# rgovindjee/mpconstellation

Measured on AMD Instinct MI355X. Metric: satellite-MPC-steps/sec (whole constellation; 1 step = discretize + constraint terms + solve per SCP iteration; inputs and results resident in HBM -- value_pcie is the same step with H2D of the inputs and D2H of the results inside), higher is better.
Workload: dtype f64

## Files before the change

### mpconstellation_amd/csrc/solve_phases.hpp

```cpp
#pragma once

namespace MPCX_NS {
#ifdef MPCX_TWO_WAVE
using namespace mpcx;
#endif

struct ResAcc {
    double dual_max, prim_max, sq, zsum, lsum, prod_min, prod_max, prod_sum;
    double g_tf;
};

struct SatData {
    double aT[8][7], bT[8];
    int nT, linvt;
    int fixed_tf;
    int shared;
    double tS, rS;
    double w_vt, gh_vt, zeta_vt;
    double b_u, b_rmax, b_rmin, b_rfmax, b_tf[2], vt_des, w_tr, w_nu, tfbar;
    double WxK[49];
    double WxKsoft[49], gxKsoft[7];
    double ta[NTERM][7], tw[NTERM], tgh[NTERM], twin[NTERM];
    double avt[7], Hv[36], cv, gam, Wtf, gtf, sigmax;
    double Mb[NBD][NBD];
    double Sb[NBD][NBD];
    double siglam[NCH], xK[NCH][7];
    double sol[NBD];
    double zeta[NTERM];
    double red[8];
    double gl[3][GL_N];
    ResAcc racc[2];
    double rs_gtf, rs_rvt, rs_gex[NTERM];
    int dir_finite;
    struct Drv {
        double mu, dw_last, E0, delta_w, alpha, tau, mu_cur, rn0, mu_clip;
        double nz, nzl;
        int n_acc, status, it_count, n_reg, first_reg, mono, refined_prev, n_small, iter, have_dir, have_trial, clean, ls;
        double tol, acc_tol;
        int acc_iter, max_iter, n_refine;
    } dv;
    static constexpr int DRV_D0 = 3, DRV_I0 = 8;
    double infeas;
    double eps_r;
    int flag;
#ifdef MPCX_PHASE_TIMING
    unsigned long long fpt[16];
#endif
};

static_assert(offsetof(SatData::Drv, mu) == 0 && offsetof(SatData::Drv, E0) == (SatData::DRV_D0 - 1) * sizeof(double) &&
              offsetof(SatData::Drv, n_small) - offsetof(SatData::Drv, n_acc) == (SatData::DRV_I0 - 1) * sizeof(int) &&
              offsetof(SatData::Drv, status) - offsetof(SatData::Drv, n_acc) == sizeof(int) &&
              offsetof(SatData::Drv, first_reg) - offsetof(SatData::Drv, n_acc) == 4 * sizeof(int), "field order of the loop state's start values");

__device__ __forceinline__ double relax(double b) { return b + kBoundRelax * fmax(1.0, fabs(b)); }

__device__ __forceinline__ double wave_max(double v)
{
#pragma unroll
    for (int o = 32; o > 0; o >>= 1) v = fmax(v, __shfl_xor(v, o, 64));
    return v;
}
__device__ __forceinline__ double wave_min(double v)
{
#pragma unroll
    for (int o = 32; o > 0; o >>= 1) v = fmin(v, __shfl_xor(v, o, 64));
    return v;
}
__device__ __forceinline__ double wave_sum(double v)
{
#pragma unroll
    for (int o = 32; o > 0; o >>= 1) v += __shfl_xor(v, o, 64);
    return v;
}

__device__ __forceinline__ double gshfl8(double v, int q)
{
    switch (q) {
    case 0: return bcast8<0>(v);
    case 1: return bcast8<1>(v);
    case 2: return bcast8<2>(v);
    case 3: return bcast8<3>(v);
    case 4: return bcast8<4>(v);
    case 5: return bcast8<5>(v);
    case 6: return bcast8<6>(v);
    default: return bcast8<7>(v);
    }
}

__device__ __forceinline__ void wsync()
{
    __builtin_amdgcn_fence(__ATOMIC_ACQ_REL, "wavefront");
    __builtin_amdgcn_wave_barrier();
}

__device__ __forceinline__ int uni(int v) { return __builtin_amdgcn_readfirstlane(v); }
__device__ __forceinline__ double uni(double v)
{
    const unsigned long long u = (unsigned long long)__double_as_longlong(v);
    const unsigned lo = __builtin_amdgcn_readfirstlane((unsigned)u), hi = __builtin_amdgcn_readfirstlane((unsigned)(u >> 32));
    return __longlong_as_double((long long)(((unsigned long long)hi << 32) | lo));
}

__device__ void vt_reduced(const double *x, double vt_des, double &c, double *g6, double *H36)
{
    const double *r = x, *v = x + 3;
    const double q = r[0] * r[0] + r[1] * r[1] + r[2] * r[2];
    const double rv = r[0] * v[0] + r[1] * v[1] + r[2] * v[2];
    const double iq = 1.0 / q, iq2 = iq * iq, iq3 = iq2 * iq;
    c = v[0] * v[0] + v[1] * v[1] + v[2] * v[2] - rv * rv * iq - vt_des * vt_des;
    if (!g6) return;
    for (int i = 0; i < 3; ++i) {
        g6[i] = -2.0 * rv * v[i] * iq + 2.0 * rv * rv * r[i] * iq2;
        g6[3 + i] = 2.0 * v[i] - 2.0 * rv * r[i] * iq;
    }
    if (!H36) return;
    for (int i = 0; i < 3; ++i)
        for (int j = 0; j < 3; ++j) {
            const double I = (i == j) ? 1.0 : 0.0;
            const double Hvv = 2.0 * I - 2.0 * r[i] * r[j] * iq;
            const double Hrr = -2.0 * v[i] * v[j] * iq + 4.0 * rv * (v[i] * r[j] + r[i] * v[j]) * iq2 +
                               2.0 * rv * rv * I * iq2 - 8.0 * rv * rv * r[i] * r[j] * iq3;
            const double Hrv = -2.0 * v[i] * r[j] * iq - 2.0 * rv * I * iq + 4.0 * rv * r[i] * r[j] * iq2;
            H36[i * 6 + j] = Hrr;
            H36[(3 + i) * 6 + 3 + j] = Hvv;
            H36[i * 6 + 3 + j] = Hrv;
            H36[(3 + j) * 6 + i] = Hrv;
        }
}

__device__ __noinline__ void build_terminal(const double *xK, double mu_grav, double r_des, const SolveOpts &o, SatData &sd)
{
    double r[3] = {xK[0], xK[1], xK[2]}, v[3] = {xK[3], xK[4], xK[5]}, h[3], rh[3], hh[3];
    const double rn = sqrt(r[0] * r[0] + r[1] * r[1] + r[2] * r[2]);
    h[0] = r[1] * v[2] - r[2] * v[1]; h[1] = r[2] * v[0] - r[0] * v[2]; h[2] = r[0] * v[1] - r[1] * v[0];
    const double hn = sqrt(h[0] * h[0] + h[1] * h[1] + h[2] * h[2]);
    for (int i = 0; i < 3; ++i) { rh[i] = r[i] / rn; hh[i] = h[i] / hn; }
    const double ihn = 1.0 / hn, ihn3 = 1.0 / (hn * hn * hn), irn = 1.0 / rn, irn3 = 1.0 / (rn * rn * rn);
    double Ph[9], hh3[9], nSv[9], Sr[9], Dr_h[9], Dv_h[9], Dr_r[9];
    for (int i = 0; i < 3; ++i)
        for (int j = 0; j < 3; ++j) {
            hh3[i * 3 + j] = ihn3 * (h[i] * h[j]);
            Ph[i * 3 + j] = (i == j ? ihn : 0.0) - hh3[i * 3 + j];
            Dr_r[i * 3 + j] = (i == j ? irn : 0.0) - irn3 * (r[i] * r[j]);
        }
    nSv[0] = 0; nSv[1] = v[2]; nSv[2] = -v[1]; nSv[3] = -v[2]; nSv[4] = 0; nSv[5] = v[0]; nSv[6] = v[1]; nSv[7] = -v[0]; nSv[8] = 0;
    Sr[0] = 0; Sr[1] = -r[2]; Sr[2] = r[1]; Sr[3] = r[2]; Sr[4] = 0; Sr[5] = -r[0]; Sr[6] = -r[1]; Sr[7] = r[0]; Sr[8] = 0;
    for (int i = 0; i < 3; ++i)
        for (int j = 0; j < 3; ++j) {
            double a = 0.0, b = 0.0;
            for (int l = 0; l < 3; ++l) { a += Ph[i * 3 + l] * nSv[l * 3 + j]; b += hh3[i * 3 + l] * Sr[l * 3 + j]; }
            Dr_h[i * 3 + j] = a;
            Dv_h[i * 3 + j] = (i == j ? ihn : 0.0) - b;
        }
    double DrVr[3], DrVn[3], DvVn[3];
    for (int j = 0; j < 3; ++j) {
        DrVr[j] = v[0] * Dr_r[j] + v[1] * Dr_r[3 + j] + v[2] * Dr_r[6 + j];
        DrVn[j] = v[0] * Dr_h[j] + v[1] * Dr_h[3 + j] + v[2] * Dr_h[6 + j];
        DvVn[j] = hh[j] + (v[0] * Dv_h[j] + v[1] * Dv_h[3 + j] + v[2] * Dv_h[6 + j]);
    }
    const double Vr = v[0] * rh[0] + v[1] * rh[1] + v[2] * rh[2];
    const double Vn = v[0] * hh[0] + v[1] * hh[1] + v[2] * hh[2];
    double gR[6] = {DrVr[0], DrVr[1], DrVr[2], rh[0], rh[1], rh[2]};
    double gN[6] = {DrVn[0], DrVn[1], DrVn[2], DvVn[0], DvVn[1], DvVn[2]};
    double gRbar = 0.0, gNbar = 0.0;
    for (int i = 0; i < 6; ++i) { gRbar += gR[i] * xK[i]; gNbar += gN[i] * xK[i]; }
    for (int i = 0; i < 8; ++i) { sd.bT[i] = 0.0; for (int j = 0; j < 7; ++j) sd.aT[i][j] = 0.0; }
    sd.linvt = o.linvt; sd.nT = o.linvt ? 8 : 6; sd.fixed_tf = o.fixed_tf | o.shared_tf; sd.shared = o.shared_tf;
    sd.w_vt = 0.0; sd.gh_vt = 0.0; sd.zeta_vt = 0.0;
    for (int j = 0; j < 3; ++j) sd.aT[0][j] = -rh[j];
    sd.bT[0] = relax(-(r_des - o.eps_r));
    for (int j = 0; j < 6; ++j) { sd.aT[1][j] = gR[j]; sd.aT[2][j] = -gR[j]; sd.aT[3][j] = gN[j]; sd.aT[4][j] = -gN[j]; }
    const double c0r = Vr - gRbar, c0n = Vn - gNbar;
    sd.bT[1] = relax(o.eps_vr - c0r); sd.bT[2] = relax(o.eps_vr + c0r);
    sd.bT[3] = relax(o.eps_vn - c0n); sd.bT[4] = relax(o.eps_vn + c0n);
    sd.aT[5][6] = -1.0; sd.bT[5] = relax(-o.min_mass);
    if (o.linvt) {
        double th[3] = {hh[1] * rh[2] - hh[2] * rh[1], hh[2] * rh[0] - hh[0] * rh[2], hh[0] * rh[1] - hh[1] * rh[0]};
        double nSrh[9] = {0, rh[2], -rh[1], -rh[2], 0, rh[0], rh[1], -rh[0], 0};
        double Shh[9] = {0, -hh[2], hh[1], hh[2], 0, -hh[0], -hh[1], hh[0], 0};
        double Dr_t[9], Dv_t[9];
        for (int i = 0; i < 3; ++i)
            for (int j = 0; j < 3; ++j) {
                double a = 0.0, b = 0.0, c = 0.0;
                for (int l = 0; l < 3; ++l) { a += nSrh[i * 3 + l] * Dr_h[l * 3 + j]; b += Shh[i * 3 + l] * Dr_r[l * 3 + j]; c += nSrh[i * 3 + l] * Dv_h[l * 3 + j]; }
                Dr_t[i * 3 + j] = a + b; Dv_t[i * 3 + j] = c;
            }
        const double Vt = v[0] * th[0] + v[1] * th[1] + v[2] * th[2];
        const double Vc = sqrt(mu_grav / rn);
        const double kc = -0.5 * sqrt(mu_grav) * pow(rn, -2.5);
        double gT[6], gbar = 0.0, DrVc_r = 0.0;
        for (int j = 0; j < 3; ++j) {
            gT[j] = v[0] * Dr_t[j] + v[1] * Dr_t[3 + j] + v[2] * Dr_t[6 + j];
            gT[3 + j] = th[j] + (v[0] * Dv_t[j] + v[1] * Dv_t[3 + j] + v[2] * Dv_t[6 + j]);
        }
        for (int i = 0; i < 6; ++i) gbar += gT[i] * xK[i];
        for (int j = 0; j < 3; ++j) { DrVc_r += kc * r[j] * r[j]; gT[j] -= kc * r[j]; }
        const double c0t = Vt - gbar - Vc + DrVc_r;
        for (int j = 0; j < 6; ++j) { sd.aT[6][j] = gT[j]; sd.aT[7][j] = -gT[j]; }
        sd.bT[6] = relax(o.eps_vt - c0t); sd.bT[7] = relax(o.eps_vt + c0t);
    }
    sd.b_u = relax(o.u_max * o.u_max);
    sd.b_rmax = relax(o.r_max * o.r_max);
    sd.b_rmin = relax(-o.r_min);
    sd.b_rfmax = relax((r_des + o.eps_r) * (r_des + o.eps_r));
    sd.b_tf[0] = relax(0.0); sd.b_tf[1] = relax(o.tf_max);
    sd.vt_des = sqrt(mu_grav / r_des);
    sd.w_tr = o.w_tr; sd.w_nu = o.w_nu;
}

__device__ __noinline__ void build_terminal_sat(const double *xK, double mu_grav, double r_des, const SolveOpts &o, const double *popts, int sat, SatData &sd)
{
    SolveOpts os = o;
    if (popts) {
// ... 658 lines not shown
            sigmax = fmax(sigmax, sig);
        }
        sd.Wtf = W; sd.gtf = g; sd.sigmax = sigmax;
    }
    WG_SYNC();
}

__device__ __noinline__ void combine_channels(const Sat &s_in, SatData &sd, int lane, bool first)
{
    double *const stg = stage_area();
    const Sat s = uniform_view(s_in);
    const int K = s.K, KP = s.KP;
    double sol[NBD];
#pragma unroll
    for (int j = 0; j < NBD; ++j) sol[j] = sd.sol[j];
    wf64 *dr = wave_uniform(s.dr);
    cwf64 *it = wave_uniform((cwf64 *)s.it);
    cgf64 *traj = wave_uniform((cgf64 *)s.traj);
    for (int k0 = 0; k0 < K; k0 += 32) {
        const int nk = (K - k0 < 32) ? K - k0 : 32;
        const int n = nk * TR_N;
        constexpr int CQ = 8;
        for (int e0 = 0; e0 < n; e0 += 64 * CQ) {
            double v[CQ];
            int slot[CQ];
#pragma unroll
            for (int q = 0; q < CQ; ++q) {
                const int e = e0 + 64 * q + lane;
                const int ec = (e < n) ? e : 0;
                const int kl = ec / TR_N, i = ec - kl * TR_N;
                cgf64 *tr = traj + (size_t)(k0 + kl) * NCH * TR_N + i;
                double acc = tr[0];
#pragma unroll
                for (int j = 0; j < NBD; ++j)
                    acc += sol[j] * tr[(1 + j) * TR_N];
                v[q] = acc; slot[q] = (e < n) ? i * CMB_LD + kl : -1;
            }
#pragma unroll
            for (int q = 0; q < CQ; ++q) if (slot[q] >= 0) stg[slot[q]] = v[q];
        }
        WG_SYNC();
        constexpr int NQ = DIR_N * 32 / 64;
        double curv[NQ], Dv[NQ], rv[NQ];
#pragma unroll
        for (int q = 0; q < NQ; ++q) {
            const int e = lane + 64 * q;
            const int i = e >> 5, kl = e & 31, k = k0 + kl;
            const int off = (i < T_U) ? I_X + i : (i < T_NU ? I_U + (i - T_U) : (i < T_LAM ? I_NU + (i - T_NU) : I_LAM + (i - T_LAM)));
            const int dst = off * KP + (kl < nk ? k : k0);
            const int kc = (kl < nk) ? k : k0, j = (i >= T_LAM) ? i - T_LAM : 0;
            curv[q] = first ? it[dst] : dr[dst];
            Dv[q] = s.nb[(size_t)kc * NB_N + N_D + j]; rv[q] = s.ch[(size_t)kc * CH_N + C_RHS + R_RHO + j];
        }
        CHUNK_END
#pragma unroll
        for (int q = 0; q < NQ; ++q) {
            const int e = lane + 64 * q;
            const int i = e >> 5, kl = e & 31, k = k0 + kl;
            const bool act = kl < nk && !(k == K - 1 && i >= T_NU);
            const int off = (i < T_U) ? I_X + i : (i < T_NU ? I_U + (i - T_U) : (i < T_LAM ? I_NU + (i - T_NU) : I_LAM + (i - T_LAM)));
            const int dst = off * KP + (kl < nk ? k : k0);
            const double cur = curv[q];
            const double base = first ? ((i >= T_LAM) ? -cur : 0.0) : cur;
            const int j = (i >= T_LAM) ? i - T_LAM : 0;
            const double val = (i >= T_LAM) ? fma(Dv[q], stg[(T_NU + j) * CMB_LD + kl], rv[q]) : stg[(i < T_LAM ? i : 0) * CMB_LD + kl];
            if (act) dr[dst] = base + val;
        }
        WG_SYNC();
    }
    if (lane == 0) {
        if (first) { s.drg[G_TF] = sd.sol[0]; s.drg[G_LVT] = sd.linvt ? 0.0 : -s.itg[G_LVT] + sd.sol[1]; }
        else { s.drg[G_TF] += sd.sol[0]; if (!sd.linvt) s.drg[G_LVT] += sd.sol[1]; }
        if (sd.linvt) sd.zeta_vt = (first ? 0.0 : sd.zeta_vt) + sd.sol[1];
        for (int t = 0; t < NTERM; ++t) sd.zeta[t] = (first ? 0.0 : sd.zeta[t]) + sd.sol[2 + t];
    }
    WG_SYNC();
}

__device__ __noinline__ void reduced_residual(const Sat &s, SatData &sd, int lane)
{
    double *const stg = stage_area();
    double rvt_rhs, gex[NTERM];
    const int K = s.K;
    double gtf_part = 0.0;
    const double dtf = s.drg[G_TF];
    double gin[NTERM], rvt_x;
    {
        const auto dKc = s.drn(K - 1);
        double dK[7];
#pragma unroll
        for (int i = 0; i < 7; ++i) dK[i] = dKc[I_X + i];
        double av = 0.0;
#pragma unroll
        for (int i = 0; i < 7; ++i) av += sd.avt[i] * dK[i];
        rvt_rhs = -sd.cv - av;
        rvt_x = rvt_rhs;
        if (sd.linvt) {
            const double wex = sd.w_vt - sd.gam;
            const bool on = wex > 0.0;
            rvt_x = -(sd.gh_vt * (sd.gam / sd.w_vt) + sd.gam * av + (on ? sd.zeta_vt : 0.0)) / sd.gam;
            rvt_rhs = on ? -(av - sd.zeta_vt / wex + sd.gh_vt / sd.w_vt) : 0.0;
        }
        for (int t = 0; t < NTERM; ++t) {
            double adx = 0.0;
#pragma unroll
            for (int i = 0; i < 7; ++i) adx += sd.ta[t][i] * dK[i];
            const double wex = sd.tw[t] - sd.twin[t];
            const double share = (sd.tw[t] > 0.0) ? sd.twin[t] / sd.tw[t] : 1.0;
            const bool on = wex > 0.0;
            gin[t] = sd.tgh[t] * share + sd.twin[t] * adx + (on ? sd.zeta[t] : 0.0);
            gex[t] = on ? (adx - sd.zeta[t] / wex + sd.tgh[t] / sd.tw[t]) * wex : 0.0;
        }
    }
    for (int k0 = 0; k0 < K; k0 += 64) {
      const int k = k0 + lane;
      double *rec = stg + lane * RHS_LD;
      if (k < K) {
        cwf64 *nb = s.nb + (size_t)k * NB_N;
        const auto ns = s.nsn(k);
        const auto p = s.itn(k), d = s.drn(k);
        const bool hp = (k >= 1), dyn = (k <= K - 2), term = (k == K - 1);
        const auto pm = p.node(hp ? -1 : 0), dm = d.node(hp ? -1 : 0), dn = d.node(dyn ? 1 : 0);
        double lt[7], ltm[7];
#pragma unroll
        for (int i = 0; i < 7; ++i) {
            const double a0 = p[I_LAM + i], a1 = d[I_LAM + i], b0 = pm[I_LAM + i], b1 = dm[I_LAM + i];
            lt[i] = dyn ? a0 + a1 : 0.0;
            ltm[i] = hp ? b0 + b1 : 0.0;
        }
        CHUNK_END
        double dx[7], du[3], dnu[7], nsgx[7], nsgu[3], w3[9], wu[9], sx[SX_N];
#pragma unroll
        for (int i = 0; i < 7; ++i) { dx[i] = d[I_X + i]; dnu[i] = d[I_NU + i]; nsgx[i] = ns[NS_GX + i]; }
#pragma unroll
        for (int i = 0; i < 3; ++i) { du[i] = d[I_U + i]; nsgu[i] = ns[NS_GU + i]; }
#pragma unroll
        for (int i = 0; i < 9; ++i) { w3[i] = nb[N_W3 + i]; wu[i] = nb[N_WU + i]; }
#pragma unroll
        for (int i = 0; i < SX_N; ++i) sx[i] = nb[N_SX + i];
        const double dg = nb[N_DIAG];
        CHUNK_END
        double gx[7], gu[3];
        if (hp) {
            if (term) {
#pragma unroll
                for (int i = 0; i < 7; ++i) {
                    double acc = sd.gxKsoft[i] + ltm[i];
#pragma unroll
                    for (int j = 0; j < 7; ++j) acc += sd.WxKsoft[i * 7 + j] * dx[j];
                    gx[i] = acc;
                }
            } else {
#pragma unroll
                for (int i = 0; i < 7; ++i) {
                    double acc = nsgx[i] + ltm[i];
                    if (i < 3) {
#pragma unroll
                        for (int j = 0; j < 3; ++j) acc += w3[i * 3 + j] * dx[j];
                    } else acc += dg * dx[i];
                    gx[i] = acc;
                }
            }
            if (term) {
                const double lvt = s.itg[G_LVT] + s.drg[G_LVT];
#pragma unroll
                for (int i = 0; i < 7; ++i) gx[i] += sd.avt[i] * lvt;
            }
        } else {
#pragma unroll
            for (int i = 0; i < 7; ++i) gx[i] = 0.0;
        }
#pragma unroll
        for (int i = 0; i < 3; ++i) {
            double acc = nsgu[i];
#pragma unroll
            for (int j = 0; j < 3; ++j) acc += wu[i * 3 + j] * du[j];
            gu[i] = acc;
        }
        {
            const double ex_x = sx[SX_EX], ex_u = sx[SX_EU];
            const double a0 = sx[SX_A], a1 = sx[SX_A + 1], a2 = sx[SX_A + 2];
            const double c0 = sx[SX_CU], c1 = sx[SX_CU + 1], c2 = sx[SX_CU + 2];
            const double px = ex_x * (a0 * dx[0] + a1 * dx[1] + a2 * dx[2]);
            const double pu = ex_u * (c0 * du[0] + c1 * du[1] + c2 * du[2]);
            if (hp && dyn) { gx[0] += px * a0; gx[1] += px * a1; gx[2] += px * a2; }
            gu[0] += pu * c0; gu[1] += pu * c1; gu[2] += pu * c2;
        }
        double sg[7], dnx[7], dnuu[3];
        {
            double bm[21];
            const auto Bm = s.Bpt(hp ? k - 1 : 0), Sg = s.Sigt(dyn ? k : 0);
#pragma unroll
            for (int e = 0; e < 21; ++e) bm[e] = Bm[e];
#pragma unroll
            for (int i = 0; i < 7; ++i) { sg[i] = Sg[i]; dnx[i] = dn[I_X + i]; }
#pragma unroll
            for (int i = 0; i < 3; ++i) dnuu[i] = dn[I_U + i];
            CHUNK_END
            if (hp) {
#pragma unroll
                for (int j = 0; j < 3; ++j) {
                    double acc = 0.0;
#pragma unroll
                    for (int i = 0; i < 7; ++i) acc += bm[i * 3 + j] * ltm[i];
                    gu[j] -= acc;
                }
            }
        }
        double aff[7], atl[7];
#pragma unroll
        for (int j = 0; j < 7; ++j) atl[j] = 0.0;
        {
            const auto A = s.At(dyn ? k : 0);
#pragma unroll
            for (int h = 0; h < 2; ++h) {
                const int r0 = h ? 4 : 0, r1 = h ? 7 : 4;
                double am[28];
#pragma unroll
                for (int i = r0; i < r1; ++i)
#pragma unroll
                    for (int j = 0; j < 7; ++j) am[(i - r0) * 7 + j] = A[i * 7 + j];
                CHUNK_END
#pragma unroll
                for (int i = r0; i < r1; ++i) {
#pragma unroll
                    for (int j = 0; j < 7; ++j) atl[j] += am[(i - r0) * 7 + j] * lt[i];
                    double acc = dnx[i] - sg[i] * dtf - dnu[i];
#pragma unroll
                    for (int j = 0; j < 7; ++j) acc -= am[(i - r0) * 7 + j] * dx[j];
                    aff[i] = acc;
                }
            }
        }
        if (dyn && hp) {
#pragma unroll
            for (int j = 0; j < 7; ++j) gx[j] -= atl[j];
        }
        {
            double bn[21], bp[21];
            const auto Bn = s.Bnt(dyn ? k : 0), Bp = s.Bpt(dyn ? k : 0);
#pragma unroll
            for (int e = 0; e < 21; ++e) { bn[e] = Bn[e]; bp[e] = Bp[e]; }
            CHUNK_END
#pragma unroll
            for (int j = 0; j < 3; ++j) {
                double acc = 0.0;
#pragma unroll
                for (int i = 0; i < 7; ++i) acc += bn[i * 3 + j] * lt[i];
                if (dyn) gu[j] -= acc;
            }
#pragma unroll
            for (int i = 0; i < 7; ++i) {
                double acc = aff[i];
#pragma unroll
                for (int j = 0; j < 3; ++j) acc -= bn[i * 3 + j] * du[j] + bp[i * 3 + j] * dnuu[j];
                aff[i] = acc;
            }
        }
        {
            double rho[7], dd[7], ee[7];
#pragma unroll
            for (int i = 0; i < 7; ++i) { rho[i] = ns[NS_RHO + i]; dd[i] = ns[NS_D + i]; ee[i] = ns[NS_E + i]; }
            CHUNK_END
            if (dyn) {
                double sl = 0.0;
#pragma unroll
                for (int i = 0; i < 7; ++i) {
                    rec[R_RHO + i] = rho[i] + dd[i] * dnu[i] - lt[i];
                    rec[R_AFF + i] = -ee[i] - aff[i];
                    sl += sg[i] * lt[i];
                }
                gtf_part -= sl;
            }
        }
        if (term) {
            for (int t = 0; t < NTERM; ++t) {
#pragma unroll
                for (int i = 0; i < 7; ++i) gx[i] += gin[t] * sd.ta[t][i];
            }
#pragma unroll
            for (int i = 0; i < 7; ++i) gx[i] -= sd.gam * rvt_x * sd.avt[i];
#pragma unroll
            for (int i = 0; i < 7; ++i) { rec[R_RHO + i] = 0.0; rec[R_AFF + i] = 0.0; }
        }
#pragma unroll
        for (int i = 0; i < 7; ++i) rec[R_GX + i] = gx[i];
#pragma unroll
        for (int i = 0; i < 3; ++i) rec[R_GU + i] = gu[i];
      }
      WG_SYNC();
      {
          const int nr = ((K - k0 < 64) ? K - k0 : 64) * RHS_N;
          wf64 *ch = s.ch + (size_t)k0 * CH_N + C_RHS;
          for (int e = lane; e < nr; e += 64) { const int kl = e / RHS_N, i = e - kl * RHS_N; ch[(size_t)kl * CH_N + i] = stg[kl * RHS_LD + i]; }
      }
      WG_SYNC();
    }
    sd.rs_gtf = sd.gtf + sd.Wtf * dtf + wave_sum(gtf_part);
    sd.rs_rvt = rvt_rhs;
#pragma unroll
    for (int t = 0; t < NTERM; ++t) sd.rs_gex[t] = gex[t];
    WG_SYNC();
}

__device__ __forceinline__ void first_rhs_scalars(SatData &sd)
{
    sd.rs_gtf = sd.gtf;
    sd.rs_rvt = sd.linvt ? -sd.gh_vt / sd.w_vt : -sd.cv;
    for (int t = 0; t < NTERM; ++t) {
        const double share = (sd.tw[t] > 0.0) ? sd.twin[t] / sd.tw[t] : 1.0;
        sd.rs_gex[t] = sd.tgh[t] * (1.0 - share);
    }
    wsync();
}

__device__ __noinline__ double finish_direction(const Sat &s, SatData &sd, double mu, double tau, int lane)
{
    const int K = s.K;
    double amax = 1.0, bad = 0.0;
#define CHK(v) { if (!(fabs(v) < 1e300)) bad = 1.0; }
    const double b_u = sd.b_u, b_rmax = sd.b_rmax, b_rmin = sd.b_rmin, w_nu = sd.w_nu;
#define LIM(v, dv) { const double v_ = (v), d_ = (dv); if (d_ < 0.0) amax = fmin(amax, -tau * v_ / d_); }
    const int half = HALF_OF(lane);
    const bool h0 = (half == 0);
    for (int k = NODE_OF(lane); k < K; k += 32) {
        const auto p = s.itn(k), d = s.drn(k);
        const auto rb = s.rbn(k);
        double x[7], dx[7], u[3], du[3], bs[6], rv[4][8];
#pragma unroll
        for (int i = 0; i < 7; ++i) { x[i] = p[I_X + i]; dx[i] = d[I_X + i]; }
#pragma unroll
        for (int i = 0; i < 3; ++i) { u[i] = p[I_U + i]; du[i] = d[I_U + i]; }
#pragma unroll
        for (int i = 0; i < 6; ++i) bs[i] = p[I_SU + i];
        const double rb0 = rb[0], rb1 = rb[1], rb2 = rb[2];
#pragma unroll
        for (int r = 0; r < 4; ++r) {
            const int iv = 4 * half + r;
            const int i = (iv < 7) ? iv : 6;
            rv[r][0] = p[I_NU + i]; rv[r][1] = p[I_T + i]; rv[r][2] = p[I_STP + i]; rv[r][3] = p[I_ZTP + i];
            rv[r][4] = p[I_STN + i]; rv[r][5] = p[I_ZTN + i]; rv[r][6] = d[I_NU + i]; rv[r][7] = d[I_LAM + i];
        }
        CHUNK_END
        {
#pragma unroll
            for (int i = 0; i < 7; ++i) CHK(dx[i]);
#pragma unroll
            for (int i = 0; i < 3; ++i) CHK(du[i]);
            {
                const PairDir q = pair_dir(bs[0], bs[1], u[0] * u[0] + u[1] * u[1] + u[2] * u[2] - b_u,
                                           2.0 * (u[0] * du[0] + u[1] * du[1] + u[2] * du[2]), mu);
                LIM(bs[0], q.ds); LIM(bs[1], q.dz);
            }
            if (k >= 1) {
                const PairDir q = pair_dir(bs[2], bs[3], x[0] * x[0] + x[1] * x[1] + x[2] * x[2] - b_rmax,
                                           2.0 * (x[0] * dx[0] + x[1] * dx[1] + x[2] * dx[2]), mu);
                LIM(bs[2], q.ds); LIM(bs[3], q.dz);
            }
            if (k >= 1 && k <= K - 2) {
                const PairDir q = pair_dir(bs[4], bs[5], -(rb0 * x[0] + rb1 * x[1] + rb2 * x[2]) - b_rmin,
                                           -(rb0 * dx[0] + rb1 * dx[1] + rb2 * dx[2]), mu);
                LIM(bs[4], q.ds); LIM(bs[5], q.dz);
            }
        }
        {
            const bool dyn = (k <= K - 2);
#pragma unroll
            for (int r = 0; r < 4; ++r) {
                const int iv = 4 * half + r;
                const bool valid = (iv < 7) && dyn;
                const double nu = rv[r][0], tt = rv[r][1], stp = rv[r][2], ztp = rv[r][3];
                const double stn = rv[r][4], ztn = rv[r][5], dnu = rv[r][6], dlam = rv[r][7];
                const L1Dir q = l1_dir(nu, tt, stp, ztp, stn, ztn, dnu, mu, w_nu);
                if (valid) {
                    CHK(dnu); CHK(dlam); CHK(q.dt);
                    LIM(stp, q.dstp); LIM(ztp, q.dztp);
                    LIM(stn, q.dstn); LIM(ztn, q.dztn);
                }
            }
        }
        if (h0 && k == K - 1) {
// ... 38 lines not shown
```

### mpconstellation_amd/csrc/solve_riccati.hpp

```cpp
#pragma once

namespace MPCX_NS {
__device__ __forceinline__ bool inv3_spd(const double *Q, double *Qi)
{
    const double a = Q[0], b = Q[1], c = Q[2], d = Q[4], e = Q[5], f = Q[8];
    const double d1 = a;
    const double r1 = rcp_pos(d1 > 0.0 ? d1 : 1.0);
    const double l21 = b * r1, l31 = c * r1;
    const double d2 = d - l21 * b;
    const double r2 = rcp_pos(d2 > 0.0 ? d2 : 1.0);
    const double t32 = e - l31 * b;
    const double l32 = t32 * r2;
    const double d3 = f - l31 * c - l32 * t32;
    const double r3 = rcp_pos(d3 > 0.0 ? d3 : 1.0);
    const bool ok = (d1 > 0.0) && (d2 > 0.0) && (d3 > 0.0);
    const double m31 = l21 * l32 - l31, m32 = -l32, m21 = -l21;
    Qi[0] = r1 + m21 * m21 * r2 + m31 * m31 * r3;
    Qi[1] = m21 * r2 + m31 * m32 * r3;
    Qi[2] = m31 * r3;
    Qi[4] = r2 + m32 * m32 * r3;
    Qi[5] = m32 * r3;
    Qi[8] = r3;
    Qi[3] = Qi[1]; Qi[6] = Qi[2]; Qi[7] = Qi[5];
    return ok;
// ... 948 lines not shown
        }
        wsync();
        FT_MARK(14)
    }
    siglam += __shfl_xor(siglam, 1, 8);
    siglam += __shfl_xor(siglam, 2, 8);
    siglam += __shfl_xor(siglam, 4, 8);
    if (act && r == 0) sd.siglam[c] = siglam;
    WG_SYNC();
}

__device__ __forceinline__ int border_channel(int q) { return q == NBD - 1 ? 1 : 2 + q; }
__device__ __forceinline__ double border_iw(const SatData &sd, int p, bool &eq)
{
    eq = (p == 0) && !sd.linvt;
    const double wex = (p == 0) ? (sd.linvt ? sd.w_vt - sd.gam : 0.0) : sd.tw[p - 1] - sd.twin[p - 1];
    return (!eq && wex > 0.0) ? 1.0 / wex : 0.0;
}

__device__ __noinline__ bool border_factor(SatData &sd, int lane)
{
    if (lane < NBD * NBD) {
        const int p = lane / NBD, q = lane - NBD * p;
        const int c = border_channel(q);
        double v;
        if (p < NBD - 1) {
            const double *a = (p == 0) ? sd.avt : sd.ta[p - 1];
            v = 0.0;
#pragma unroll
            for (int l = 0; l < 7; ++l) v += a[l] * sd.xK[c][l];
        } else v = (q == NBD - 1 ? sd.Wtf : 0.0) - sd.siglam[c];
        if (sd.fixed_tf && (p == NBD - 1 || q == NBD - 1)) v = (p == q) ? 1.0 : 0.0;
        sd.Mb[p][q] = v; sd.Sb[p][q] = v;
    }
    WG_SYNC();
    double S[NBD][NBD];
#pragma unroll
    for (int p = 0; p < NBD; ++p)
#pragma unroll
        for (int q = 0; q < NBD; ++q) S[p][q] = sd.Mb[p][q];
#pragma unroll
    for (int p = 0; p < NBD - 1; ++p) {
        bool eq;
        const double iw = border_iw(sd, p, eq);
        const bool on = iw > 0.0;
        if (eq) continue;
#pragma unroll
        for (int q = 0; q < NBD; ++q) if (!on && q != p) { S[p][q] = 0.0; S[q][p] = 0.0; }
        S[p][p] = on ? S[p][p] - iw : -1.0;
    }
    bool ok = true;
    double rd[NBD];
#pragma unroll
    for (int p = 0; p < NBD; ++p) {
        const double d = S[p][p];
        if (p == NBD - 1) { if (!(d > 0.0)) ok = false; } else if (!(d < 0.0)) ok = false;
        rd[p] = 1.0 / d;
#pragma unroll
        for (int i = p + 1; i < NBD; ++i) {
            const double m = S[i][p] * rd[p];
#pragma unroll
            for (int j = p + 1; j < NBD; ++j) S[i][j] -= m * S[p][j];
            S[i][p] = m;
        }
    }
    WG_SYNC();
    if (lane == 0) {
#pragma unroll
        for (int p = 0; p < NBD; ++p) {
            sd.Mb[p][p] = rd[p];
#pragma unroll
            for (int i = p + 1; i < NBD; ++i) sd.Mb[i][p] = S[i][p];
        }
    }
    WG_SYNC();
    return ok;
}

__device__ __noinline__ void border_solve(SatData &sd, int lane)
{
    const double gtf_rhs = sd.rs_gtf, rvt_rhs = sd.rs_rvt;
    const double *gex = sd.rs_gex;
    double rb[NBD], x[NBD], r[NBD];
#pragma unroll
    for (int p = 0; p < NBD - 1; ++p) {
        const double *a = (p == 0) ? sd.avt : sd.ta[p - 1];
        double acc = 0.0;
#pragma unroll
        for (int l = 0; l < 7; ++l) acc += a[l] * sd.xK[0][l];
        rb[p] = -acc;
    }
    rb[0] += rvt_rhs;
    double iw[NBD - 1];
    bool eqr[NBD - 1];
#pragma unroll
    for (int p = 0; p < NBD - 1; ++p) {
        iw[p] = border_iw(sd, p, eqr[p]);
        if (p >= 1) rb[p] = (iw[p] > 0.0) ? rb[p] - gex[p - 1] * iw[p] : 0.0;
        else if (!eqr[0] && !(iw[0] > 0.0)) rb[0] = 0.0;
    }
    rb[NBD - 1] = sd.fixed_tf ? 0.0 : -gtf_rhs + sd.siglam[0];
    auto ldl_solve = [&](double (&v)[NBD]) {
#pragma unroll
        for (int p = 0; p < NBD; ++p)
#pragma unroll
            for (int i = p + 1; i < NBD; ++i) v[i] -= sd.Mb[i][p] * v[p];
#pragma unroll
        for (int p = 0; p < NBD; ++p) v[p] *= sd.Mb[p][p];
#pragma unroll
        for (int p = NBD - 1; p >= 0; --p)
#pragma unroll
            for (int i = p + 1; i < NBD; ++i) v[p] -= sd.Mb[i][p] * v[i];
    };
#pragma unroll
    for (int p = 0; p < NBD; ++p) x[p] = rb[p];
    ldl_solve(x);
#pragma unroll
    for (int p = 0; p < NBD; ++p) {
        double acc = rb[p];
#pragma unroll
        for (int q = 0; q < NBD; ++q) {
            double s = sd.Sb[p][q];
            const int pc = p < NBD - 1 ? p : 0, qc = q < NBD - 1 ? q : 0;
            const bool zp = p < NBD - 1 && !eqr[pc], zq = q < NBD - 1 && !eqr[qc];
            const bool offp = zp && !(iw[pc] > 0.0), offq = zq && !(iw[qc] > 0.0);
            if (p == q && zp) s = offp ? -1.0 : s - iw[pc];
            else if (offp || offq) s = 0.0;
            acc -= s * x[q];
        }
        r[p] = acc;
    }
    ldl_solve(r);
#pragma unroll
    for (int p = 0; p < NBD; ++p) x[p] += r[p];
    WG_SYNC();
    if (lane == 0) {
        sd.sol[0] = x[NBD - 1];
#pragma unroll
        for (int p = 0; p < NBD - 1; ++p) sd.sol[1 + p] = x[p];
    }
    WG_SYNC();
}


constexpr long kSpinMax = 20000000;
struct GridSync {
    double *red;
    int32_t *arrive, *abort_flag;
    int S, blk, phase;
    bool aborted;
};

__device__ __noinline__ void grid_reduce(GridSync &g, double (&v)[GR_N], int lane)
{
    double *slot = g.red + ((size_t)(g.phase & 1) * g.S + g.blk) * GR_N;
    if (lane == 0) {
#pragma unroll
        for (int j = 0; j < GR_N; ++j) __hip_atomic_store(slot + j, v[j], __ATOMIC_RELAXED, __HIP_MEMORY_SCOPE_AGENT);
    }
    __threadfence();
    WG_SYNC();
    if (lane == 0) {
        __hip_atomic_fetch_add(g.arrive, 1, __ATOMIC_RELEASE, __HIP_MEMORY_SCOPE_AGENT);
        const int target = (g.phase + 1) * g.S;
        long spins = 0;
        while (__hip_atomic_load(g.arrive, __ATOMIC_ACQUIRE, __HIP_MEMORY_SCOPE_AGENT) < target) {
            if (__hip_atomic_load(g.abort_flag, __ATOMIC_RELAXED, __HIP_MEMORY_SCOPE_AGENT) != 0) break;
            if (++spins > kSpinMax) { __hip_atomic_store(g.abort_flag, 1, __ATOMIC_RELAXED, __HIP_MEMORY_SCOPE_AGENT); break; }
            __builtin_amdgcn_s_sleep(16);
        }
    }
    WG_SYNC();
    __threadfence();
// ... 173 lines not shown
```

Before: 779,800.

## Split per-node residual work across two half-waves and parallelize border RHS dots

The reduced residual loop now maps one node to a lane pair instead of one lane, covering 32 nodes per pass. The lower half-wave computes the gradient terms (gx, gu) and the upper half computes the dynamics affine and rho residuals, sharing one A-matrix pass through transposed indexing. The gtf partial sum is kept in even/odd accumulators and combined across halves with a shuffle. Separately, the border solve computes its NBD-1 dot products one per lane and broadcasts them with readlane, and build_terminal is forced inline. This raises per-lane parallelism and shortens each lane's serial chain, at the cost of twice as many loop passes and staging rounds, some duplicated loads, and divergent branches.

Measured after the change: 804,800, median of 6. +3.2%, better.

```diff
diff --git a/mpconstellation_amd/csrc/solve_phases.hpp b/mpconstellation_amd/csrc/solve_phases.hpp
--- a/mpconstellation_amd/csrc/solve_phases.hpp
+++ b/mpconstellation_amd/csrc/solve_phases.hpp
@@ -102,6 +102,13 @@
     return __longlong_as_double((long long)(((unsigned long long)hi << 32) | lo));
 }
 
+__device__ __forceinline__ double lane_value(double v, int l)
+{
+    const unsigned long long u = (unsigned long long)__double_as_longlong(v);
+    const unsigned lo = __builtin_amdgcn_readlane((unsigned)u, l), hi = __builtin_amdgcn_readlane((unsigned)(u >> 32), l);
+    return __longlong_as_double((long long)(((unsigned long long)hi << 32) | lo));
+}
+
 __device__ void vt_reduced(const double *x, double vt_des, double &c, double *g6, double *H36)
 {
     const double *r = x, *v = x + 3;
@@ -129,7 +136,7 @@
         }
 }
 
-__device__ __noinline__ void build_terminal(const double *xK, double mu_grav, double r_des, const SolveOpts &o, SatData &sd)
+__device__ __forceinline__ void build_terminal(const double *xK, double mu_grav, double r_des, const SolveOpts &o, SatData &sd)
 {
     double r[3] = {xK[0], xK[1], xK[2]}, v[3] = {xK[3], xK[4], xK[5]}, h[3], rh[3], hh[3];
     const double rn = sqrt(r[0] * r[0] + r[1] * r[1] + r[2] * r[2]);
@@ -954,7 +961,6 @@
     double *const stg = stage_area();
     double rvt_rhs, gex[NTERM];
     const int K = s.K;
-    double gtf_part = 0.0;
     const double dtf = s.drg[G_TF];
     double gin[NTERM], rvt_x;
     {
@@ -984,191 +990,220 @@
             gex[t] = on ? (adx - sd.zeta[t] / wex + sd.tgh[t] / sd.tw[t]) * wex : 0.0;
         }
     }
-    for (int k0 = 0; k0 < K; k0 += 64) {
-      const int k = k0 + lane;
-      double *rec = stg + lane * RHS_LD;
+    const int half = HALF_OF(lane), kl = NODE_OF(lane);
+    const bool h0 = (half == 0);
+    double gtf_even = 0.0, gtf_odd = 0.0;
+    for (int k0 = 0; k0 < K; k0 += 32) {
+      const int k = k0 + kl;
+      double *rec = stg + kl * RHS_LD;
       if (k < K) {
-        cwf64 *nb = s.nb + (size_t)k * NB_N;
-        const auto ns = s.nsn(k);
         const auto p = s.itn(k), d = s.drn(k);
         const bool hp = (k >= 1), dyn = (k <= K - 2), term = (k == K - 1);
         const auto pm = p.node(hp ? -1 : 0), dm = d.node(hp ? -1 : 0), dn = d.node(dyn ? 1 : 0);
-        double lt[7], ltm[7];
-#pragma unroll
-        for (int i = 0; i < 7; ++i) {
-            const double a0 = p[I_LAM + i], a1 = d[I_LAM + i], b0 = pm[I_LAM + i], b1 = dm[I_LAM + i];
-            lt[i] = dyn ? a0 + a1 : 0.0;
-            ltm[i] = hp ? b0 + b1 : 0.0;
-        }
-        CHUNK_END
-        double dx[7], du[3], dnu[7], nsgx[7], nsgu[3], w3[9], wu[9], sx[SX_N];
-#pragma unroll
-        for (int i = 0; i < 7; ++i) { dx[i] = d[I_X + i]; dnu[i] = d[I_NU + i]; nsgx[i] = ns[NS_GX + i]; }
-#pragma unroll
-        for (int i = 0; i < 3; ++i) { du[i] = d[I_U + i]; nsgu[i] = ns[NS_GU + i]; }
-#pragma unroll
-        for (int i = 0; i < 9; ++i) { w3[i] = nb[N_W3 + i]; wu[i] = nb[N_WU + i]; }
-#pragma unroll
-        for (int i = 0; i < SX_N; ++i) sx[i] = nb[N_SX + i];
-        const double dg = nb[N_DIAG];
-        CHUNK_END
+        double lt[7];
+        double q0[7], q1[7];
+        {
+            double a0[7], a1[7], b0[7], b1[7];
+#pragma unroll
+            for (int i = 0; i < 7; ++i) { a0[i] = p[I_LAM + i]; a1[i] = d[I_LAM + i]; }
+            if (h0) {
+#pragma unroll
+                for (int i = 0; i < 7; ++i) { b0[i] = pm[I_LAM + i]; b1[i] = dm[I_LAM + i]; }
+            } else {
+#pragma unroll
+                for (int i = 0; i < 7; ++i) { b0[i] = dn[I_X + i]; b1[i] = d[I_NU + i]; }
+            }
+            CHUNK_END
+#pragma unroll
+            for (int i = 0; i < 7; ++i) {
+                lt[i] = dyn ? a0[i] + a1[i] : 0.0;
+                const double ltm = hp ? b0[i] + b1[i] : 0.0;
+                q0[i] = h0 ? ltm : b0[i]; q1[i] = b1[i];
+            }
+        }
+        double dx[7], du[3];
         double gx[7], gu[3];
-        if (hp) {
-            if (term) {
-#pragma unroll
-                for (int i = 0; i < 7; ++i) {
-                    double acc = sd.gxKsoft[i] + ltm[i];
-#pragma unroll
-                    for (int j = 0; j < 7; ++j) acc += sd.WxKsoft[i * 7 + j] * dx[j];
-                    gx[i] = acc;
+        double out[7], vec[7];
+        double dnuu[3];
+#pragma unroll
+        for (int i = 0; i < 7; ++i) dx[i] = d[I_X + i];
+#pragma unroll
+        for (int i = 0; i < 3; ++i) du[i] = d[I_U + i];
+        if (h0) {
+            cwf64 *nb = s.nb + (size_t)k * NB_N;
+            const auto ns = s.nsn(k);
+            double nsgx[7], nsgu[3], w3[9], wu[9], sx[SX_N];
+#pragma unroll
+            for (int i = 0; i < 7; ++i) nsgx[i] = ns[NS_GX + i];
+#pragma unroll
+            for (int i = 0; i < 3; ++i) nsgu[i] = ns[NS_GU + i];
+#pragma unroll
+            for (int i = 0; i < 9; ++i) { w3[i] = nb[N_W3 + i]; wu[i] = nb[N_WU + i]; }
+#pragma unroll
+            for (int i = 0; i < SX_N; ++i) sx[i] = nb[N_SX + i];
+            const double dg = nb[N_DIAG];
+            CHUNK_END
+            const double *ltm = q0;
+            if (hp) {
+                if (term) {
+#pragma unroll
+                    for (int i = 0; i < 7; ++i) {
+                        double acc = sd.gxKsoft[i] + ltm[i];
+#pragma unroll
+                        for (int j = 0; j < 7; ++j) acc += sd.WxKsoft[i * 7 + j] * dx[j];
+                        gx[i] = acc;
+                    }
+                } else {
+#pragma unroll
+                    for (int i = 0; i < 7; ++i) {
+                        double acc = nsgx[i] + ltm[i];
+                        if (i < 3) {
+#pragma unroll
+                            for (int j = 0; j < 3; ++j) acc += w3[i * 3 + j] * dx[j];
+                        } else acc += dg * dx[i];
+                        gx[i] = acc;
+                    }
+                }
+                if (term) {
+                    const double lvt = s.itg[G_LVT] + s.drg[G_LVT];
+#pragma unroll
+                    for (int i = 0; i < 7; ++i) gx[i] += sd.avt[i] * lvt;
                 }
             } else {
 #pragma unroll
-                for (int i = 0; i < 7; ++i) {
-                    double acc = nsgx[i] + ltm[i];
-                    if (i < 3) {
-#pragma unroll
-                        for (int j = 0; j < 3; ++j) acc += w3[i * 3 + j] * dx[j];
-                    } else acc += dg * dx[i];
-                    gx[i] = acc;
-                }
-            }
-            if (term) {
-                const double lvt = s.itg[G_LVT] + s.drg[G_LVT];
-#pragma unroll
-                for (int i = 0; i < 7; ++i) gx[i] += sd.avt[i] * lvt;
-            }
+                for (int i = 0; i < 7; ++i) gx[i] = 0.0;
+            }
+#pragma unroll
+            for (int i = 0; i < 3; ++i) {
+                double acc = nsgu[i];
+#pragma unroll
+                for (int j = 0; j < 3; ++j) acc += wu[i * 3 + j] * du[j];
+                gu[i] = acc;
+            }
+            {
+                const double ex_x = sx[SX_EX], ex_u = sx[SX_EU];
+                const double a0 = sx[SX_A], a1 = sx[SX_A + 1], a2 = sx[SX_A + 2];
+                const double c0 = sx[SX_CU], c1 = sx[SX_CU + 1], c2 = sx[SX_CU + 2];
+                const double px = ex_x * (a0 * dx[0] + a1 * dx[1] + a2 * dx[2]);
+                const double pu = ex_u * (c0 * du[0] + c1 * du[1] + c2 * du[2]);
+                if (hp && dyn) { gx[0] += px * a0; gx[1] += px * a1; gx[2] += px * a2; }
+                gu[0] += pu * c0; gu[1] += pu * c1; gu[2] += pu * c2;
+            }
+#pragma unroll
+            for (int i = 0; i < 7; ++i) { out[i] = 0.0; vec[i] = lt[i]; }
         } else {
-#pragma unroll
-            for (int i = 0; i < 7; ++i) gx[i] = 0.0;
-        }
-#pragma unroll
-        for (int i = 0; i < 3; ++i) {
-            double acc = nsgu[i];
-#pragma unroll
-            for (int j = 0; j < 3; ++j) acc += wu[i * 3 + j] * du[j];
-            gu[i] = acc;
-        }
-        {
-            const double ex_x = sx[SX_EX], ex_u = sx[SX_EU];
-            const double a0 = sx[SX_A], a1 = sx[SX_A + 1], a2 = sx[SX_A + 2];
-            const double c0 = sx[SX_CU], c1 = sx[SX_CU + 1], c2 = sx[SX_CU + 2];
-            const double px = ex_x * (a0 * dx[0] + a1 * dx[1] + a2 * dx[2]);
-            const double pu = ex_u * (c0 * du[0] + c1 * du[1] + c2 * du[2]);
-            if (hp && dyn) { gx[0] += px * a0; gx[1] += px * a1; gx[2] += px * a2; }
-            gu[0] += pu * c0; gu[1] += pu * c1; gu[2] += pu * c2;
-        }
-        double sg[7], dnx[7], dnuu[3];
-        {
-            double bm[21];
-            const auto Bm = s.Bpt(hp ? k - 1 : 0), Sg = s.Sigt(dyn ? k : 0);
-#pragma unroll
-            for (int e = 0; e < 21; ++e) bm[e] = Bm[e];
-#pragma unroll
-            for (int i = 0; i < 7; ++i) { sg[i] = Sg[i]; dnx[i] = dn[I_X + i]; }
+            const auto ns = s.nsn(k);
+            const auto Sg = s.Sigt(dyn ? k : 0);
+            double sg[7], rho[7], dd[7];
+#pragma unroll
+            for (int i = 0; i < 7; ++i) { sg[i] = Sg[i]; rho[i] = ns[NS_RHO + i]; dd[i] = ns[NS_D + i]; }
 #pragma unroll
             for (int i = 0; i < 3; ++i) dnuu[i] = dn[I_U + i];
             CHUNK_END
-            if (hp) {
-#pragma unroll
-                for (int j = 0; j < 3; ++j) {
-                    double acc = 0.0;
-#pragma unroll
-                    for (int i = 0; i < 7; ++i) acc += bm[i * 3 + j] * ltm[i];
-                    gu[j] -= acc;
-                }
-            }
-        }
-        double aff[7], atl[7];
-#pragma unroll
-        for (int j = 0; j < 7; ++j) atl[j] = 0.0;
+            const double *dnx = q0, *dnu = q1;
+#pragma unroll
+            for (int i = 0; i < 7; ++i) { out[i] = dnx[i] - sg[i] * dtf - dnu[i]; vec[i] = -dx[i]; }
+            if (dyn) {
+                double sl = 0.0;
+#pragma unroll
+                for (int i = 0; i < 7; ++i) {
+                    rec[R_RHO + i] = rho[i] + dd[i] * dnu[i] - lt[i];
+                    sl += sg[i] * lt[i];
+                }
+                if (k0 & 32) gtf_odd -= sl; else gtf_even -= sl;
+            }
+        }
         {
             const auto A = s.At(dyn ? k : 0);
+            const int ra = h0 ? 7 : 1, rb = h0 ? 1 : 7;
 #pragma unroll
             for (int h = 0; h < 2; ++h) {
                 const int r0 = h ? 4 : 0, r1 = h ? 7 : 4;
                 double am[28];
 #pragma unroll
-                for (int i = r0; i < r1; ++i)
-#pragma unroll
-                    for (int j = 0; j < 7; ++j) am[(i - r0) * 7 + j] = A[i * 7 + j];
+                for (int a = r0; a < r1; ++a)
+#pragma unroll
+                    for (int b = 0; b < 7; ++b) am[(a - r0) * 7 + b] = A[a * ra + b * rb];
                 CHUNK_END
 #pragma unroll
-                for (int i = r0; i < r1; ++i) {
-#pragma unroll
-                    for (int j = 0; j < 7; ++j) atl[j] += am[(i - r0) * 7 + j] * lt[i];
-                    double acc = dnx[i] - sg[i] * dtf - dnu[i];
-#pragma unroll
-                    for (int j = 0; j < 7; ++j) acc -= am[(i - r0) * 7 + j] * dx[j];
-                    aff[i] = acc;
-                }
-            }
-        }
-        if (dyn && hp) {
-#pragma unroll
-            for (int j = 0; j < 7; ++j) gx[j] -= atl[j];
+                for (int a = r0; a < r1; ++a)
+#pragma unroll
+                    for (int b = 0; b < 7; ++b) out[b] += am[(a - r0) * 7 + b] * vec[a];
+            }
+        }
+        if (h0) {
+            if (dyn && hp) {
+#pragma unroll
+                for (int j = 0; j < 7; ++j) gx[j] -= out[j];
+            }
+            if (term) {
+                for (int t = 0; t < NTERM; ++t) {
+#pragma unroll
+                    for (int i = 0; i < 7; ++i) gx[i] += gin[t] * sd.ta[t][i];
+                }
+#pragma unroll
+                for (int i = 0; i < 7; ++i) gx[i] -= sd.gam * rvt_x * sd.avt[i];
+            }
+#pragma unroll
+            for (int i = 0; i < 7; ++i) rec[R_GX + i] = gx[i];
         }
         {
-            double bn[21], bp[21];
-            const auto Bn = s.Bnt(dyn ? k : 0), Bp = s.Bpt(dyn ? k : 0);
+            double bn[21], bp[21], ee[7];
+            const auto Bn = s.Bnt(dyn ? k : 0), Bp = s.Bpt(h0 ? (hp ? k - 1 : 0) : (dyn ? k : 0));
 #pragma unroll
             for (int e = 0; e < 21; ++e) { bn[e] = Bn[e]; bp[e] = Bp[e]; }
+            if (!h0) {
+                const auto ns = s.nsn(k);
+#pragma unroll
+                for (int i = 0; i < 7; ++i) ee[i] = ns[NS_E + i];
+            }
             CHUNK_END
-#pragma unroll
-            for (int j = 0; j < 3; ++j) {
-                double acc = 0.0;
-#pragma unroll
-                for (int i = 0; i < 7; ++i) acc += bn[i * 3 + j] * lt[i];
-                if (dyn) gu[j] -= acc;
-            }
-#pragma unroll
-            for (int i = 0; i < 7; ++i) {
-                double acc = aff[i];
-#pragma unroll
-                for (int j = 0; j < 3; ++j) acc -= bn[i * 3 + j] * du[j] + bp[i * 3 + j] * dnuu[j];
-                aff[i] = acc;
-            }
-        }
-        {
-            double rho[7], dd[7], ee[7];
-#pragma unroll
-            for (int i = 0; i < 7; ++i) { rho[i] = ns[NS_RHO + i]; dd[i] = ns[NS_D + i]; ee[i] = ns[NS_E + i]; }
-            CHUNK_END
-            if (dyn) {
-                double sl = 0.0;
+            if (h0) {
+                const double *ltm = q0;
+                if (hp) {
+#pragma unroll
+                    for (int j = 0; j < 3; ++j) {
+                        double acc = 0.0;
+#pragma unroll
+                        for (int i = 0; i < 7; ++i) acc += bp[i * 3 + j] * ltm[i];
+                        gu[j] -= acc;
+                    }
+                }
+#pragma unroll
+                for (int j = 0; j < 3; ++j) {
+                    double acc = 0.0;
+#pragma unroll
+                    for (int i = 0; i < 7; ++i) acc += bn[i * 3 + j] * lt[i];
+                    if (dyn) gu[j] -= acc;
+                }
+#pragma unroll
+                for (int i = 0; i < 3; ++i) rec[R_GU + i] = gu[i];
+            } else {
 #pragma unroll
                 for (int i = 0; i < 7; ++i) {
-                    rec[R_RHO + i] = rho[i] + dd[i] * dnu[i] - lt[i];
-                    rec[R_AFF + i] = -ee[i] - aff[i];
-                    sl += sg[i] * lt[i];
-                }
-                gtf_part -= sl;
-            }
-        }
-        if (term) {
-            for (int t = 0; t < NTERM; ++t) {
-#pragma unroll
-                for (int i = 0; i < 7; ++i) gx[i] += gin[t] * sd.ta[t][i];
-            }
-#pragma unroll
-            for (int i = 0; i < 7; ++i) gx[i] -= sd.gam * rvt_x * sd.avt[i];
-#pragma unroll
-            for (int i = 0; i < 7; ++i) { rec[R_RHO + i] = 0.0; rec[R_AFF + i] = 0.0; }
-        }
-#pragma unroll
-        for (int i = 0; i < 7; ++i) rec[R_GX + i] = gx[i];
-#pragma unroll
-        for (int i = 0; i < 3; ++i) rec[R_GU + i] = gu[i];
+                    double acc = out[i];
+#pragma unroll
+                    for (int j = 0; j < 3; ++j) acc -= bn[i * 3 + j] * du[j] + bp[i * 3 + j] * dnuu[j];
+                    if (dyn) rec[R_AFF + i] = -ee[i] - acc;
+                }
+                if (term) {
+#pragma unroll
+                    for (int i = 0; i < 7; ++i) { rec[R_RHO + i] = 0.0; rec[R_AFF + i] = 0.0; }
+                }
+            }
+        }
       }
       WG_SYNC();
       {
-          const int nr = ((K - k0 < 64) ? K - k0 : 64) * RHS_N;
+          const int nr = ((K - k0 < 32) ? K - k0 : 32) * RHS_N;
           wf64 *ch = s.ch + (size_t)k0 * CH_N + C_RHS;
-          for (int e = lane; e < nr; e += 64) { const int kl = e / RHS_N, i = e - kl * RHS_N; ch[(size_t)kl * CH_N + i] = stg[kl * RHS_LD + i]; }
+          for (int e = lane; e < nr; e += 64) { const int kr = e / RHS_N, i = e - kr * RHS_N; ch[(size_t)kr * CH_N + i] = stg[kr * RHS_LD + i]; }
       }
       WG_SYNC();
     }
-    sd.rs_gtf = sd.gtf + sd.Wtf * dtf + wave_sum(gtf_part);
+    const double gtf_below = __shfl_xor(gtf_even, 32, 64);
+    const double gtf_lane = h0 ? gtf_below : gtf_odd;
+    sd.rs_gtf = sd.gtf + sd.Wtf * dtf + wave_sum(gtf_lane);
     sd.rs_rvt = rvt_rhs;
 #pragma unroll
     for (int t = 0; t < NTERM; ++t) sd.rs_gex[t] = gex[t];
diff --git a/mpconstellation_amd/csrc/solve_riccati.hpp b/mpconstellation_amd/csrc/solve_riccati.hpp
--- a/mpconstellation_amd/csrc/solve_riccati.hpp
+++ b/mpconstellation_amd/csrc/solve_riccati.hpp
@@ -1054,13 +1054,15 @@
     const double gtf_rhs = sd.rs_gtf, rvt_rhs = sd.rs_rvt;
     const double *gex = sd.rs_gex;
     double rb[NBD], x[NBD], r[NBD];
-#pragma unroll
-    for (int p = 0; p < NBD - 1; ++p) {
-        const double *a = (p == 0) ? sd.avt : sd.ta[p - 1];
+    {
+        const int pl = (lane < NBD - 1) ? lane : 0;
+        const double *a = (pl == 0) ? sd.avt : sd.ta[pl - 1];
         double acc = 0.0;
 #pragma unroll
         for (int l = 0; l < 7; ++l) acc += a[l] * sd.xK[0][l];
-        rb[p] = -acc;
+        const double nacc = -acc;
+#pragma unroll
+        for (int p = 0; p < NBD - 1; ++p) rb[p] = lane_value(nacc, p);
     }
     rb[0] += rvt_rhs;
     double iw[NBD - 1];
```
